# freemvmt/two-towers-overlords

Measured on NVIDIA B200. Metric: train_triplets_per_sec, higher is better.
Workload: dtype f32 (bf16x3 tensor-core projection)

## Files before the change

### two-towers-overlords_b200/csrc/tt_chain_sm100.cu

```cuda
#include <stdlib.h>

#include "tt_ptx.cuh"
#include "tt_step_ws.cuh"
#include "tt_tma.cuh"

namespace tt {

namespace {

using namespace ptx;

constexpr int BM = 128, BN = 128, BK = 64;
constexpr int kMaxStages = 6;
constexpr int kAcc = 4;
constexpr int kEpiThreads = 256;
constexpr int kThreads = 64 + kEpiThreads;
constexpr uint32_t kABytes = BM * BK * 2, kBBytes = BN * BK * 2, kStageBytes = kABytes + kBBytes;
constexpr int kSplitPad = 66;
constexpr int kRowStage = 3072;
constexpr int kTermPitch = 48;
constexpr int kTermBlock = 32 * kTermPitch;
constexpr int kF32Pitch = 80;
constexpr int kCsBytes = 2 * 8 * 64 * 4;
constexpr int kStagingBytes = kCsBytes  + 8 * kRowStage  + 64;
static_assert(2 * 64 * kSplitPad * 2 <= 8 * kRowStage, "split tiles overlay the row staging");
constexpr size_t chain_smem(int stages) { return (size_t)stages * kStageBytes + 1024 + 256 + kStagingBytes; }
constexpr float kCosEps = 1e-8f;
constexpr long long kSpinLimit = 4000000000ll;

enum { T_S = 0, T_T, T_F1, T_F2L, T_DZ, T_DX, T_DW2, T_DW1, T_G, T_COUNT };

struct TowerMaps {
  CUtensorMap x[3], w1[3];
  CUtensorMap h[2], w2[2];
  CUtensorMap dy[2];
  CUtensorMap dz[2], w1k[2];
  CUtensorMap dyk[2], hk[2];
  CUtensorMap dzk[2], xk[2];
};

struct SplitJobC {
  const float* X;
  bf16 *hi, *lo, *lo2;
  int R, C;
  int f4_0;
};

struct alignas(64) ChainParams {
  TowerMaps tm[2];
  int B, H, P, RTB, NC, NCH, NCF;
  int pairs, terms, pairs1, terms1;
  int kcb, nch[2], kbt[2];
  int off[T_COUNT + 1];
  int stages, n_sj, n_split_f4, n_split_f4_w1;
  int nS;
  int use_pdl;
  SplitJobC sj[6];
  float margin, inv_batch, grad_scale;
  const float *b1[2], *b2[2];
  float *h, *y, *dy, *dz1, *dxhat, *stats, *loss;
  bf16 *h_hi, *h_lo, *dy_hi, *dy_lo, *dz_hi, *dz_lo;
  float *part2, *part1;
  float *dW1[2], *db1[2], *dW2[2], *db2[2];
  float *stat_part, *cs1, *cs2, *hinge_part, *ybuf;
  unsigned* ctr;
  int n_counters;
  double* adam_state;
  float *adam_p, *adam_g, *adam_m, *adam_v;
  float lr, beta1, beta2, eps;
  int grad_accumulate;
  unsigned total_signals, dw2_signals;
  unsigned long long* trace;
};

__device__ __forceinline__ unsigned ld_acquire(const unsigned* p) {
  unsigned v;
  asm volatile("ld.acquire.gpu.global.u32 %0, [%1];" : "=r"(v) : "l"(p) : "memory");
  return v;
}
// ... 34 lines not shown
};
__device__ __forceinline__ RowTile row_tile(const ChainParams& p, int u) {
  RowTile rt;
  rt.r = u / 3;
  rt.seg = u - 3 * rt.r;
  rt.t = rt.seg != 0;
  rt.trow = (rt.seg == 2 ? p.B : 0) + rt.r * BM;
  rt.grow = rt.seg * p.B + rt.r * BM;
  rt.valid = min(BM, p.B - rt.r * BM);
  return rt;
}

struct Sub {
  const CUtensorMap *a, *b;
  int terms, pairs, m0, n0, kb0, nkb;
  int bn;
  int amn, bmn;
};
__device__ __forceinline__ int n_subs(int type) {
  return (type == T_S || type == T_T || type == T_G) ? 0 : 1;
}

__device__ __forceinline__ void dw_chunk(const ChainParams& p, int ci, int& t, int& j) {
  t = ci >= p.nch[0];
  j = ci - (t ? p.nch[0] : 0);
}

__device__ __forceinline__ Sub get_sub(const ChainParams& p, Task tk, int k) {
  Sub s;
  s.terms = p.terms;
  s.pairs = p.pairs;
  s.kb0 = 0;
  s.bn = BN;
  s.amn = s.bmn = 0;
  switch (tk.type) {
    case T_F1: {
      const RowTile rt = row_tile(p, tk.i / p.NC);
      s.a = p.tm[rt.t].x; s.b = p.tm[rt.t].w1;
      s.terms = p.terms1; s.pairs = p.pairs1;
      s.m0 = rt.trow; s.n0 = (tk.i % p.NC) * BN; s.nkb = p.H / BK;
    } break;
    case T_F2L: {
      const int seg = tk.i % 3, rc = tk.i / 3, r = rc / p.NCF, t = seg != 0;
      s.a = p.tm[t].h; s.b = p.tm[t].w2;
      s.m0 = (seg == 2 ? p.B : 0) + r * BM; s.n0 = (rc % p.NCF) * 64; s.nkb = p.P / BK;
      s.bn = 64;
    } break;
    case T_DZ: {
      const RowTile rt = row_tile(p, tk.i / p.NC);
      s.a = p.tm[rt.t].dy; s.b = p.tm[rt.t].w2; s.bmn = 1;
      s.m0 = rt.trow; s.n0 = (tk.i % p.NC) * BN; s.nkb = p.P / BK;
    } break;
    case T_DX: {
      const RowTile rt = row_tile(p, tk.i / p.NCH);
      s.a = p.tm[rt.t].dz; s.b = p.tm[rt.t].w1k; s.bmn = 1;
      s.m0 = rt.trow; s.n0 = (tk.i % p.NCH) * BN; s.nkb = p.P / BK;
    } break;
    case T_DW2: {
      const int nt_ = p.NC * p.NC, tile = tk.i % nt_;
      int t, j;
      dw_chunk(p, tk.i / nt_, t, j);
      s.a = p.tm[t].dyk; s.b = p.tm[t].hk; s.amn = s.bmn = 1;
      s.m0 = (tile / p.NC) * BM; s.n0 = (tile % p.NC) * BN;
      s.kb0 = j * p.kcb; s.nkb = min(p.kcb, p.kbt[t] - s.kb0);
    } break;
    default: {
      const int nt_ = p.NC * p.NCH, tile = tk.i % nt_;
      int t, j;
      dw_chunk(p, tk.i / nt_, t, j);
      s.a = p.tm[t].dzk; s.b = p.tm[t].xk; s.amn = s.bmn = 1;
      s.m0 = (tile / p.NCH) * BM; s.n0 = (tile % p.NCH) * BN;
      s.kb0 = j * p.kcb; s.nkb = min(p.kcb, p.kbt[t] - s.kb0);
    } break;
  }
  return s;
}

__device__ __forceinline__ unsigned* h_ready(const ChainParams& p) { return p.ctr + 8; }
__device__ __forceinline__ unsigned* dy_ready(const ChainParams& p) { return p.ctr + 8 + 3 * p.RTB; }
__device__ __forceinline__ unsigned* dz_ready(const ChainParams& p) { return p.ctr + 8 + 6 * p.RTB; }
__device__ __forceinline__ unsigned* stat_ready(const ChainParams& p) { return p.ctr + 8 + 9 * p.RTB; }
__device__ __forceinline__ unsigned* y_ready(const ChainParams& p) { return p.ctr + 8 + 10 * p.RTB; }

__device__ __forceinline__ void wait_rows(const ChainParams& p, const unsigned* ready, unsigned need, int t, int k0,
                                          int k1) {
  if (t == 0) {
    for (int r = k0 / BM; r <= (k1 - 1) / BM; ++r) wait_counter(ready + r, need);
    return;
  }
  if (k0 < p.B)
    for (int r = k0 / BM; r <= (min(k1, p.B) - 1) / BM; ++r) wait_counter(ready + p.RTB + r, need);
  if (k1 > p.B)
    for (int r = (max(k0, p.B) - p.B) / BM; r <= (k1 - p.B - 1) / BM; ++r) wait_counter(ready + 2 * p.RTB + r, need);
}

__device__ __forceinline__ void wait_deps(const ChainParams& p, Task tk) {
  switch (tk.type) {
    case T_F1: wait_counter(p.ctr + 0, (unsigned)p.nS); break;
    case T_F2L: {
      const int seg = tk.i % 3, r = tk.i / 3 / p.NCF;
      wait_counter(p.ctr + 2, (unsigned)p.nS);
      wait_counter(h_ready(p) + seg * p.RTB + r, p.NC);
    } break;
    case T_DZ: {
      const RowTile rt = row_tile(p, tk.i / p.NC);
      wait_counter(dy_ready(p) + rt.seg * p.RTB + rt.r, p.NCF);
    } break;
    case T_DX: {
      const RowTile rt = row_tile(p, tk.i / p.NCH);
      wait_counter(dz_ready(p) + rt.seg * p.RTB + rt.r, p.NC);
    } break;
    case T_DW2:
    case T_DW1: {
      const int nt_ = tk.type == T_DW2 ? p.NC * p.NC : p.NC * p.NCH;
      int t, j;
      dw_chunk(p, tk.i / nt_, t, j);
      const int k0 = j * p.kcb * BK, k1 = min(k0 + p.kcb * BK, t ? 2 * p.B : p.B);
      if (tk.type == T_DW2) wait_rows(p, dy_ready(p), p.NCF, t, k0, k1);
      else wait_rows(p, dz_ready(p), p.NC, t, k0, k1);
    } break;
    default: break;
  }
}

__device__ __forceinline__ float colsum16(const float (&v)[16], int lane) {
  float a[8], b[4], c[2];
  const bool h16 = lane & 16, h8 = lane & 8, h4 = lane & 4, h2 = lane & 2;
#pragma unroll
  for (int j = 0; j < 8; ++j) {
    const float keep = h16 ? v[8 + j] : v[j], send = h16 ? v[j] : v[8 + j];
    a[j] = keep + __shfl_xor_sync(0xffffffffu, send, 16);
  }
#pragma unroll
// ... 82 lines not shown
  e.ab += n;
  if (e.ab >= kAcc) {
    e.ab -= kAcc;
    e.aph ^= 1u;
  }
}
__device__ __forceinline__ void publish(const EpiCtx& e) {
  fence_proxy_async();
  __threadfence();
  epi_bar();
}

__device__ __forceinline__ void stage_cs(const EpiCtx& e, int slot, int chunk, float d) {
  if ((e.lane & 1) == 0) e.cs_s[(slot * 8 + e.we) * 64 + chunk * 16 + (e.lane >> 1)] = d;
}
__device__ __forceinline__ float reduce_cs(const EpiCtx& e, int slot, int col, int cw = 64) {
  const int hf = col / cw, cc = col - hf * cw;
  float s = 0.f;
#pragma unroll
  for (int quarter = 0; quarter < 4; ++quarter) s += e.cs_s[(slot * 8 + hf * 4 + ((quarter - 2) & 3)) * 64 + cc];
  return s;
}

__device__ __forceinline__ uint32_t pack_bf16(bf16 a, bf16 b) {
  return (uint32_t)__bfloat16_as_ushort(a) | ((uint32_t)__bfloat16_as_ushort(b) << 16);
}

__device__ void epi_split(const ChainParams& p, EpiCtx& e, int task_i) {
  const int nS = p.nS;
  if (task_i == 0 && e.tid == 0 && p.adam_state) {
    const double t = p.adam_state[0];
    p.adam_state[0] = t + 1.0;
// ... 73 lines not shown
    stage16(e.rs, e.lane, hi);
    stage16(e.rs + kTermBlock, e.lane, lo);
    if (ok && p.h) store16(p.h + (wrow0 + e.lane) * p.P + n, v);
    __syncwarp();
    flush16(e.rs, e.lane, p.h_hi, wrow0, n, p.P, vr);
    flush16(e.rs + kTermBlock, e.lane, p.h_lo, wrow0, n, p.P, vr);
    __syncwarp();
  }
  tc_fence_before();
  mbar_arrive(&e.acc_empty[e.ab]);
  acc_advance(e, 1);
  publish(e);
  if (e.tid == 0) signal(h_ready(p) + rt.seg * p.RTB + rt.r);
}

__device__ void epi_f2l(const ChainParams& p, EpiCtx& e, int task_i) {
  const int seg = task_i % 3, rc = task_i / 3, r = rc / p.NCF, c = rc % p.NCF, n0 = c * 64;
  const int valid = min(BM, p.B - r * BM);
  const int row = e.q * 32 + e.lane;
  const bool ok = row < valid;
  const int vr = warp_valid_rows(e, valid);
  const int trip = r * BM + row;
  const size_t wrow0 = (size_t)seg * p.B + (size_t)r * BM + e.q * 32;
  mbar_wait(&e.acc_full[e.ab], e.aph);
  tc_fence_after();
  trace_ev(e, 2);
  const uint32_t accb = e.tmem_base + ((uint32_t)(e.q * 32) << 16) + (uint32_t)(e.ab * BN + e.hf * 32);
  const float* bias = p.b2[seg != 0];
  float* X = p.ybuf + (size_t)rc * 3 * 64 * 128;
  float own[32];
#pragma unroll
  for (int ch = 0; ch < 2; ++ch) {
    const int col = e.hf * 32 + ch * 16;
    float v[16];
    tmem_ld16(accb + ch * 16, v);
#pragma unroll
    for (int j = 0; j < 16; ++j) {
      v[j] += __ldg(bias + n0 + col + j);
      own[ch * 16 + j] = v[j];
      X[((size_t)(seg * 64 + col + j)) * 128 + row] = v[j];
    }
    if (p.y && ok) store16(p.y + ((size_t)seg * p.B + trip) * p.P + n0 + col, v);
  }
  tc_fence_before();
  mbar_arrive(&e.acc_empty[e.ab]);
  acc_advance(e, 1);
  __threadfence();
  epi_bar();
  if (e.tid == 0) {
    signal(y_ready(p) + rc);
    wait_counter(y_ready(p) + rc, 3u);
  }
  epi_bar();
  const int s1 = seg == 0 ? 1 : 0, s2 = seg == 2 ? 1 : 2;
  float f1[32], f2[32];
  {
    const float* x1 = X + (size_t)(s1 * 64 + e.hf * 32) * 128 + row;
    const float* x2 = X + (size_t)(s2 * 64 + e.hf * 32) * 128 + row;
#pragma unroll
    for (int j = 0; j < 32; ++j) {
      f1[j] = __ldcg(x1 + (size_t)j * 128);
      f2[j] = __ldcg(x2 + (size_t)j * 128);
    }
  }
  float qq = 0.f, pp = 0.f, nn = 0.f, qp = 0.f, qn = 0.f;
#pragma unroll
  for (int j = 0; j < 32; ++j) {
    const float a = seg == 0 ? own[j] : f1[j];
    const float b = seg == 0 ? f1[j] : (seg == 1 ? own[j] : f2[j]);
    const float d = seg == 2 ? own[j] : f2[j];
    qq = fmaf(a, a, qq);
    pp = fmaf(b, b, pp);
    nn = fmaf(d, d, nn);
    qp = fmaf(a, b, qp);
    qn = fmaf(a, d, qn);
  }
  const int nslots = p.NCF;
  float* xs = e.cs_s;
  if (seg == 0 && e.hf == 1) {
    xs[row] = qq; xs[128 + row] = pp; xs[256 + row] = nn; xs[384 + row] = qp; xs[512 + row] = qn;
  }
  epi_bar();
  if (seg == 0 && e.hf == 0) {
    float* sp = p.stat_part + ((size_t)(r * nslots + c) * 5) * 128 + row;
    sp[0] = qq + xs[row]; sp[128] = pp + xs[128 + row]; sp[256] = nn + xs[256 + row]; sp[384] = qp + xs[384 + row];
    sp[512] = qn + xs[512 + row];
    __threadfence();
  }
  epi_bar();
  if (e.tid == 0) {
    if (seg == 0) signal(stat_ready(p) + r);
    wait_counter(stat_ready(p) + r, (unsigned)p.NCF);
  }
  epi_bar();
  trace_ev(e, 3);
  qq = pp = nn = qp = qn = 0.f;
  for (int s0 = 0; s0 < nslots; s0 += 4) {
    float v[4][5];
#pragma unroll
    for (int u = 0; u < 4; ++u) {
      const float* sp = p.stat_part + ((size_t)(r * nslots + min(s0 + u, nslots - 1)) * 5) * 128 + row;
#pragma unroll
      for (int w = 0; w < 5; ++w) v[u][w] = __ldcg(sp + 128 * w);
    }
#pragma unroll
    for (int u = 0; u < 4; ++u)
      if (s0 + u < nslots) {
        qq += v[u][0]; pp += v[u][1]; nn += v[u][2]; qp += v[u][3]; qn += v[u][4];
      }
  }
  const float nq = sqrtf(qq), np_ = sqrtf(pp), nn_ = sqrtf(nn);
  const float cq = fmaxf(nq, kCosEps), cp = fmaxf(np_, kCosEps), cn = fmaxf(nn_, kCosEps);
  const float cos_p = qp / (cq * cp), cos_n = qn / (cq * cn);
  const float hinge = ok ? fmaxf((1.f - cos_p) - (1.f - cos_n) + p.margin, 0.f) : 0.f;
  const float gh = (hinge > 0.f) ? p.grad_scale * p.inv_batch : 0.f;
  const float a_qp = -gh / (cq * cp), a_qn = gh / (cq * cn);
  float c_own, c1, c2;
  if (seg == 0) {
    c_own = -((nq > kCosEps) ? (-gh * cos_p + gh * cos_n) / (cq * nq) : 0.f); c1 = a_qp; c2 = a_qn;
  } else if (seg == 1) {
    c_own = -((np_ > kCosEps) ? (-gh * cos_p) / (cp * np_) : 0.f); c1 = a_qp; c2 = 0.f;
  } else {
    c_own = -((nn_ > kCosEps) ? (gh * cos_n) / (cn * nn_) : 0.f); c1 = a_qn; c2 = 0.f;
  }
  if (seg == 0 && c == 0 && e.hf == 0) {
    if (ok) {
      float* s = p.stats + (size_t)trip * 8;
      s[0] = cos_p; s[1] = cos_n; s[2] = hinge; s[3] = nq; s[4] = np_; s[5] = nn_; s[6] = qp; s[7] = qn;
    }
    const float hsum = warp_sum(hinge);
    if (e.lane == 0) e.hs_s[e.q] = hsum;
  }
  uint8_t* blk_hi = e.rs;
  uint8_t* blk_lo = e.rs + kTermBlock;
#pragma unroll
  for (int ch = 0; ch < 2; ++ch) {
    const int n = n0 + e.hf * 32 + ch * 16;
    float g[16];
#pragma unroll
    for (int j = 0; j < 16; ++j)
      g[j] = ok ? (c_own * own[ch * 16 + j] + c1 * f1[ch * 16 + j] + c2 * f2[ch * 16 + j]) : 0.f;
    alignas(16) bf16 hi[16], lo[16];
    split16(g, hi, lo);
    stage16(blk_hi, e.lane, hi);
    stage16(blk_lo, e.lane, lo);
    if (ok && p.dy) store16(p.dy + ((size_t)seg * p.B + trip) * p.P + n, g);
    __syncwarp();
    flush16(blk_hi, e.lane, p.dy_hi, wrow0, n, p.P, vr);
    flush16(blk_lo, e.lane, p.dy_lo, wrow0, n, p.P, vr);
    __syncwarp();
    stage_cs(e, 0, ch, colsum16(g, e.lane));
  }
  epi_bar();
  if (e.tid < 64) p.cs2[(size_t)(seg * p.RTB + r) * p.P + n0 + e.tid] = reduce_cs(e, 0, e.tid, 32);
  if (seg == 0 && c == 0 && e.tid == 0) p.hinge_part[r] = (e.hs_s[0] + e.hs_s[1]) + (e.hs_s[2] + e.hs_s[3]);
  publish(e);
  if (e.tid == 0) {
    signal(dy_ready(p) + seg * p.RTB + r);
    signal(p.ctr + 1);
  }
}

__device__ void epi_dz(const ChainParams& p, EpiCtx& e, int task_i) {
  const RowTile rt = row_tile(p, task_i / p.NC);
  const int n0 = (task_i % p.NC) * BN;
  mbar_wait(&e.acc_full[e.ab], e.aph);
  tc_fence_after();
  trace_ev(e, 2);
  const int row = e.q * 32 + e.lane;
  const bool ok = row < rt.valid;
  const int vr = warp_valid_rows(e, rt.valid);
  const size_t wrow0 = (size_t)rt.grow + e.q * 32;
  for (int ch = 0; ch < 4; ++ch) {
// ... 173 lines not shown
            if (j + c4 < nch[u]) acc[u] = add4(acc[u], t[u][c4]);
      }
      emit4(p, k, dst[0], acc[0]);
      if (two) emit4(p, k, dst[1], acc[1]);
    }
  };
  sum_pairs(p.ctr + 6, p.part2, p.dW2, (size_t)p.P * p.P / 4);
  if (e.tid == 0) wait_counter(p.ctr + 1, p.total_signals);
  epi_bar();
  sum_pairs(p.ctr + 7, p.part1, p.dW1, (size_t)p.P * p.H / 4);
  {
    const int nout = 4 * p.P;
    const int gw = task_i * 8 + e.we, nw = nG * 8;
    for (int o = gw; o < nout; o += nw) {
      const int which = o / p.P, n = o - which * p.P, t = which & 1;
      const float* src;
      int cnt;
      if (which < 2) {
        src = p.cs2 + (size_t)(t ? p.RTB : 0) * p.P + n;
        cnt = t ? 2 * p.RTB : p.RTB;
      } else {
        src = p.cs1 + (size_t)(t ? p.RTB : 0) * p.P + n;
        cnt = t ? 2 * p.RTB : p.RTB;
      }
      float s = 0.f;
      for (int r = e.lane; r < cnt; r += 32) s += __ldcg(src + (size_t)r * p.P);
      s = warp_sum(s);
      if (e.lane == 0) emit1(p, k, (which < 2 ? p.db2[t] : p.db1[t]) + n, s);
    }
  }
  if (task_i == 0 && e.tid == 0) {
    float s = 0.f;
    for (int r = 0; r < p.RTB; ++r) s += __ldcg(p.hinge_part + r);
    *p.loss = s * p.inv_batch;
  }
  epi_bar();
  if (e.tid == 0) {
    __threadfence();
    if (atomicAdd(p.ctr + 4, 1u) == (unsigned)nG - 1u) {
      for (int i = 0; i < p.n_counters; ++i) p.ctr[i] = 0u;
    }
  }
}

__global__ void __launch_bounds__(kThreads, 1) chain_kernel(const __grid_constant__ ChainParams p) {
  extern __shared__ uint8_t smem_raw[];
  const int warp = threadIdx.x >> 5, lane = threadIdx.x & 31;
  const uint32_t raw = smem_u32(smem_raw);
// ... 31 lines not shown
    if (elect_one()) {
      int s = 0;
      uint32_t ph = 0;
      if (p.use_pdl) pdl_wait();
      for (int idx = blockIdx.x; idx < n_tasks; idx += gridDim.x) {
        const Task tk = decode(p, idx);
        const int ns = n_subs(tk.type);
        if (ns == 0) continue;
        wait_deps(p, tk);
        fence_proxy_async();
        for (int k = 0; k < ns; ++k) {
          const Sub sb = get_sub(p, tk, k);
          for (int kb = sb.kb0; kb < sb.kb0 + sb.nkb; ++kb) {
            for (int j = 0; j < sb.terms; ++j) {
              mbar_wait(&empty[s], ph ^ 1u);
              mbar_arrive_expect_tx(&full[s], kABytes + (uint32_t)sb.bn * BK * 2);
              uint8_t* sa = smem + s * kStageBytes;
              uint8_t* sbm = sa + kABytes;
              if (sb.amn) {
                tma_load_2d(sa, &sb.a[j], &full[s], sb.m0, kb * BK);
                tma_load_2d(sa + kABytes / 2, &sb.a[j], &full[s], sb.m0 + 64, kb * BK);
              } else {
                tma_load_2d(sa, &sb.a[j], &full[s], kb * BK, sb.m0);
              }
              if (sb.bmn) {
                tma_load_2d(sbm, &sb.b[j], &full[s], sb.n0, kb * BK);
                tma_load_2d(sbm + kBBytes / 2, &sb.b[j], &full[s], sb.n0 + 64, kb * BK);
              } else {
                tma_load_2d(sbm, &sb.b[j], &full[s], kb * BK, sb.n0);
              }
              if (++s == NS) {
                s = 0;
                ph ^= 1u;
              }
            }
          }
        }
      }
    }
  } else if (warp == 1) {
    if (elect_one()) {
      constexpr uint32_t idesc128 = make_idesc_bf16(BM, BN), idesc64 = make_idesc_bf16(BM, 64);
      const uint32_t ring = smem_u32(smem);
      int s = 0, ab = 0;
      uint32_t ph = 0, aph = 0;
      for (int idx = blockIdx.x; idx < n_tasks; idx += gridDim.x) {
        const Task tk = decode(p, idx);
        const int ns = n_subs(tk.type);
        for (int k = 0; k < ns; ++k) {
          const Sub sb = get_sub(p, tk, k);
          const uint32_t idesc = (sb.bn == BN ? idesc128 : idesc64) | ((uint32_t)sb.amn << 15) | ((uint32_t)sb.bmn << 16);
          const uint64_t a_step = sb.amn ? 128 : 2, b_step = sb.bmn ? 128 : 2;
          mbar_wait(&acc_empty[ab], aph ^ 1u);
          tc_fence_after();
          const uint32_t acc = tmem_base + (uint32_t)(ab * BN);
          for (int kbi = 0; kbi < sb.nkb; ++kbi) {
            uint32_t slot_addr[3];
            int slot_id[3];
            for (int j = 0; j < sb.terms; ++j) {
              mbar_wait(&full[s], ph);
              slot_id[j] = s;
              slot_addr[j] = ring + (uint32_t)s * kStageBytes;
              if (++s == NS) {
                s = 0;
                ph ^= 1u;
              }
// ... 34 lines not shown
    e.tid = threadIdx.x - 64;
    e.ab = 0;
    e.aph = 0;
    e.trace = p.trace ? p.trace + (size_t)blockIdx.x * kTraceSlots * 2 : nullptr;
    e.tslot = 0;
    for (int idx = blockIdx.x; idx < n_tasks; idx += gridDim.x) {
      const Task tk = decode(p, idx);
      e.tidx = idx;
      trace_ev(e, 0);
      switch (tk.type) {
        case T_S:
          epi_split(p, e, tk.i);
          if (p.use_pdl) pdl_wait();
          break;
        case T_F1: epi_f1(p, e, tk.i); break;
        case T_F2L: epi_f2l(p, e, tk.i); break;
        case T_DZ: epi_dz(p, e, tk.i); break;
        case T_DX: epi_dx(p, e, tk.i); break;
        case T_DW2:
        case T_DW1: epi_dw(p, e, tk); break;
        default: epi_grad(p, e, tk.i); break;
      }
      trace_ev(e, 1);
    }
  }
  tc_fence_before();
  __syncthreads();
  if (warp == 1) tmem_dealloc(tmem_base, kAcc * BN);
}

constexpr int kChainStages = 5;
// ... 37 lines not shown
  const float* W2[2] = {s.Wq2, s.Wd2};
  const int row0[2] = {0, B}, rows[2] = {B, 2 * B};
  const bool x3 = s.n_split == 3;
  for (int t = 0; t < 2; ++t) {
    TowerMaps& m = p.tm[t];
    const size_t oH = (size_t)row0[t] * H, oP = (size_t)row0[t] * P;
    const bf16* x[3] = {w.x_hi + oH, x3 ? w.x_lo + oH : nullptr, x3 ? w.x_lo2 + oH : nullptr};
    const bf16* w1[3] = {w.w1_hi[t], w.w1_lo[t], w.w1_lo2[t]};
    const bf16* hh[2] = {w.h_hi + oP, w.h_lo + oP};
    const bf16* w2[2] = {w.w2_hi[t], w.w2_lo[t]};
    const bf16* dy[2] = {w.dy_hi + oP, w.dy_lo + oP};
    const bf16* dz[2] = {w.dz_hi + oP, w.dz_lo + oP};
    if ((rc = map_terms(m.x, 3, x, rows[t], H, H))) return rc;
    if ((rc = map_terms(m.w1, 3, w1, P, H, H))) return rc;
    if ((rc = map_terms(m.h, 2, hh, rows[t], P, P))) return rc;
    if ((rc = map_terms(m.w2, 2, w2, P, P, P, 64))) return rc;
    if ((rc = map_terms(m.dy, 2, dy, rows[t], P, P))) return rc;
    if ((rc = map_terms(m.dz, 2, dz, rows[t], P, P))) return rc;
    if ((rc = map_terms(m.w1k, 2, w1, P, H, H, 64))) return rc;
    if ((rc = map_terms(m.dyk, 2, dy, rows[t], P, P, 64))) return rc;
    if ((rc = map_terms(m.hk, 2, hh, rows[t], P, P, 64))) return rc;
    if ((rc = map_terms(m.dzk, 2, dz, rows[t], P, P, 64))) return rc;
    if ((rc = map_terms(m.xk, 2, x, rows[t], H, H, 64))) return rc;
  }
  p.B = B; p.H = H; p.P = P;
  p.RTB = (B + BM - 1) / BM; p.NC = (P + BN - 1) / BN; p.NCH = (H + BN - 1) / BN; p.NCF = P / 64;
  p.pairs = x3 ? 3 : 1; p.terms = x3 ? 2 : 1;
  p.pairs1 = x3 ? 6 : 1; p.terms1 = x3 ? 3 : 1;
  for (int t = 0; t < 2; ++t) p.kbt[t] = (rows[t] + BK - 1) / BK;
  p.kcb = 8;
  {
    const char* e = getenv("TT_CHAIN_KCB");
    if (e && atoi(e) >= 4) p.kcb = atoi(e) / 4 * 4;
  }
  while ((p.kbt[0] + p.kcb - 1) / p.kcb + (p.kbt[1] + p.kcb - 1) / p.kcb > 48) p.kcb += 8;
  for (int t = 0; t < 2; ++t) p.nch[t] = (p.kbt[t] + p.kcb - 1) / p.kcb;
  const int grid = sm_count();
  TT_REQUIRE(grid >= 3 * (P / 64), "tt_triplet_step: projection dim %d needs %d co-resident CTAs, the device has %d SMs", P,
             3 * (P / 64), grid);
  const int n_rt = 3 * p.RTB, nchs = p.nch[0] + p.nch[1];
  const int count[T_COUNT] = {grid,
                              0,
                              n_rt * p.NC,
                              n_rt * p.NCF,
                              n_rt * p.NC,
                              s.dxhat ? n_rt * p.NCH : 0,
                              nchs * p.NC * p.NC,
                              nchs * p.NC * p.NCH,
                              grid};
  p.off[0] = 0;
  for (int k = 0; k < T_COUNT; ++k) p.off[k + 1] = p.off[k] + count[k];
  p.total_signals = (unsigned)(count[T_F2L] + count[T_DZ] + count[T_DW2] + count[T_DW1]);
  p.dw2_signals = (unsigned)count[T_DW2];
  p.stages = kChainStages;
  int f4 = 0;
  p.n_sj = 0;
  for (int t = 0; t < 2; ++t) {
    p.sj[p.n_sj++] = SplitJobC{W1[t], w.w1_hi[t], w.w1_lo[t], x3 ? w.w1_lo2[t] : nullptr, P, H, f4};
    f4 += P * H / 4;
  }
  p.n_split_f4_w1 = f4;
  for (int t = 0; t < 2; ++t) {
    p.sj[p.n_sj++] = SplitJobC{W2[t], w.w2_hi[t], w.w2_lo[t], nullptr, P, P, f4};
    f4 += P * P / 4;
  }
  p.n_split_f4 = f4;
  p.margin = s.margin; p.inv_batch = s.inv_batch; p.grad_scale = s.grad_scale;
  p.b1[0] = s.bq1; p.b1[1] = s.bd1; p.b2[0] = s.bq2; p.b2[1] = s.bd2;
  const bool dbg = chain_debug_out() != 0;
  p.h = dbg ? s.h : nullptr; p.y = dbg ? s.y : nullptr; p.dy = dbg ? s.dy : nullptr; p.dz1 = dbg ? w.dz1 : nullptr;
  p.dxhat = s.dxhat; p.stats = s.stats; p.loss = s.loss;
  p.h_hi = w.h_hi; p.h_lo = w.h_lo;
  p.dy_hi = w.dy_hi; p.dy_lo = w.dy_lo;
  p.dz_hi = w.dz_hi; p.dz_lo = w.dz_lo;
  p.part2 = w.partial2; p.part1 = w.partial;
  p.dW1[0] = s.dWq1; p.dW1[1] = s.dWd1; p.db1[0] = s.dbq1; p.db1[1] = s.dbd1;
  p.dW2[0] = s.dWq2; p.dW2[1] = s.dWd2; p.db2[0] = s.dbq2; p.db2[1] = s.dbd2;
  p.stat_part = w.stat_part; p.cs1 = w.cs1; p.cs2 = w.cs2; p.hinge_part = w.hinge_part; p.ybuf = w.ybuf;
  p.ctr = w.counters;
  p.n_counters = w.n_counters;
  p.nS = grid;
  p.grad_accumulate = s.grad_accumulate;
  if (s.adam.param) {
    const FusedAdam& a = s.adam;
    TT_REQUIRE(a.state && a.grad && a.exp_avg && a.exp_avg_sq, "tt_triplet_step: fused Adam needs state, grad and both moments");
    const float* W[8] = {s.Wq1, s.bq1, s.Wq2, s.bq2, s.Wd1, s.bd1, s.Wd2, s.bd2};
    float* G[8] = {s.dWq1, s.dbq1, s.dWq2, s.dbq2, s.dWd1, s.dbd1, s.dWd2, s.dbd2};
    const size_t len[8] = {(size_t)P * H, (size_t)P, (size_t)P * P, (size_t)P, (size_t)P * H, (size_t)P, (size_t)P * P, (size_t)P};
    for (int i = 0; i < 8; ++i) {
      const ptrdiff_t off = G[i] - a.grad;
      TT_REQUIRE(off >= 0 && (size_t)off + len[i] <= a.n && W[i] == a.param + off && off % 4 == 0,
                 "tt_triplet_step: fused Adam wants the 8 projection tensors and their gradients to be slices of the "
                 "flat buffers at equal, 16-byte aligned offsets (tensor %d)", i);
// ... 27 lines not shown
```

### two-towers-overlords_b200/csrc/tt_step_ws.cuh

```cuda
#pragma once
#include "tt_simt.cuh"
#include "tt_sm100.cuh"

namespace tt {

using bf16 = __nv_bfloat16;
static inline int round64(int x) { return (x + 63) / 64 * 64; }

struct StepWs {
  int ldt, dcol;
  bf16 *x_hi, *x_lo, *x_lo2, *xt_hi, *xt_lo;
  bf16 *h_hi, *h_lo, *ht_hi, *ht_lo;
  bf16 *dy_hi, *dy_lo, *dyt_hi, *dyt_lo;
  bf16 *dz_hi, *dz_lo, *dzt_hi, *dzt_lo;
  bf16 *w1_hi[2], *w1_lo[2], *w1_lo2[2], *w1t_hi[2], *w1t_lo[2];
  bf16 *w2_hi[2], *w2_lo[2], *w2t_hi[2], *w2t_lo[2];
  float *dz1, *partial, *partial2, *colsum, *colsum2, *loss_scratch;
  float *stat_part, *cs1, *cs2, *hinge_part, *ybuf;
  unsigned* counters;
  int n_counters;
  unsigned long long* trace;
};
constexpr int kTraceSlots = 64, kTraceCtas = 160;

static inline size_t carve_step(char* base, int B, int H, int P, int train_table, StepWs* out) {
  char* p = base;
  StepWs w{};
  w.dcol = round64(B);
  w.ldt = w.dcol + round64(2 * B);
  const size_t R = (size_t)3 * B;
  w.x_hi = ws_take<bf16>(p, R * H); w.x_lo = ws_take<bf16>(p, R * H); w.x_lo2 = ws_take<bf16>(p, R * H);
  w.xt_hi = ws_take<bf16>(p, (size_t)H * w.ldt); w.xt_lo = ws_take<bf16>(p, (size_t)H * w.ldt);
  w.h_hi = ws_take<bf16>(p, R * P); w.h_lo = ws_take<bf16>(p, R * P);
// ... 4 lines not shown
  w.dzt_hi = ws_take<bf16>(p, (size_t)P * w.ldt); w.dzt_lo = ws_take<bf16>(p, (size_t)P * w.ldt);
  for (int t = 0; t < 2; ++t) {
    w.w1_hi[t] = ws_take<bf16>(p, (size_t)P * H); w.w1_lo[t] = ws_take<bf16>(p, (size_t)P * H);
    w.w1_lo2[t] = ws_take<bf16>(p, (size_t)P * H);
    w.w1t_hi[t] = ws_take<bf16>(p, (size_t)P * H); w.w1t_lo[t] = ws_take<bf16>(p, (size_t)P * H);
    w.w2_hi[t] = ws_take<bf16>(p, (size_t)P * P); w.w2_lo[t] = ws_take<bf16>(p, (size_t)P * P);
    w.w2t_hi[t] = ws_take<bf16>(p, (size_t)P * P); w.w2t_lo[t] = ws_take<bf16>(p, (size_t)P * P);
  }
  w.dz1 = ws_take<float>(p, R * P);
  w.partial = ws_take<float>(p, (size_t)2 * 32 * P * max(P, H));
  w.partial2 = ws_take<float>(p, (size_t)2 * 32 * P * P);
  w.colsum = ws_take<float>(p, (size_t)2 * kColsumSlices * P);
  w.colsum2 = ws_take<float>(p, (size_t)2 * kColsumSlices * P);
  w.loss_scratch = ws_take<float>(p, (size_t)(B + 3) / 4 + 8);
  {
    const int RTB = (B + 127) / 128, NC = (P + 127) / 128;
    w.stat_part = ws_take<float>(p, (size_t)RTB * 2 * (P / 64 + 1) * 5 * 128);
    w.cs1 = ws_take<float>(p, (size_t)3 * RTB * P);
    w.cs2 = ws_take<float>(p, (size_t)3 * RTB * P);
    w.ybuf = ws_take<float>(p, (size_t)3 * RTB * 128 * P);
    w.hinge_part = ws_take<float>(p, (size_t)RTB + 8);
    w.n_counters = 10 * RTB + 8 + RTB * (P / 64 + 1);
    w.counters = ws_take<unsigned>(p, (size_t)w.n_counters);
    w.trace = ws_take<unsigned long long>(p, (size_t)kTraceCtas * kTraceSlots * 2);
  }
  (void)train_table;
  if (out) *out = w;
  return (size_t)(p - base) + 256;
}


}
```

Baseline: 8.511 million.

## Split fused F2+loss task into separate F2 GEMM and per-row-block loss tasks

Replaces the fused F2L task (64-wide N tiles that exchanged y across CTAs and spun on per-row-block statistic barriers) with a plain 128-wide F2 GEMM that writes y to a column-major buffer, plus a separate loss task. The loss task waits on all three segments, reduces norms and dot products in shared memory, and emits dy for all three segments, with each row block split into quarter-row and column-part pieces. This removes the cross-CTA spin waits inside the epilogue and the need for 3*(P/64) co-resident CTAs, and it moves F2 to full 128-wide MMA tiles. In exchange the loss tasks reread y from global memory and column sums gain a fourth partial dimension.

Result: no change. 8.538 million, median of 6 (+0.3%).

```diff
diff --git a/two-towers-overlords_b200/csrc/tt_chain_sm100.cu b/two-towers-overlords_b200/csrc/tt_chain_sm100.cu
--- a/two-towers-overlords_b200/csrc/tt_chain_sm100.cu
+++ b/two-towers-overlords_b200/csrc/tt_chain_sm100.cu
@@ -27,13 +27,15 @@
 constexpr size_t chain_smem(int stages) { return (size_t)stages * kStageBytes + 1024 + 256 + kStagingBytes; }
 constexpr float kCosEps = 1e-8f;
 constexpr long long kSpinLimit = 4000000000ll;
-
-enum { T_S = 0, T_T, T_F1, T_F2L, T_DZ, T_DX, T_DW2, T_DW1, T_G, T_COUNT };
+constexpr int kLCP = 2, kLPR = 4 * kLCP;
+static_assert(5 * 8 * 32 * 4 <= 8 * kRowStage, "a round of loss statistics overlays the row staging");
+
+enum { T_S = 0, T_T, T_F1, T_F2, T_L, T_DZ, T_DX, T_DW2, T_DW1, T_G, T_COUNT };
 
 struct TowerMaps {
   CUtensorMap x[3], w1[3];
   CUtensorMap h[2], w2[2];
-  CUtensorMap dy[2];
+  CUtensorMap dy[2], w2k[2];
   CUtensorMap dz[2], w1k[2];
   CUtensorMap dyk[2], hk[2];
   CUtensorMap dzk[2], xk[2];
@@ -48,7 +50,7 @@
 
 struct alignas(64) ChainParams {
   TowerMaps tm[2];
-  int B, H, P, RTB, NC, NCH, NCF;
+  int B, H, P, RTB, NC, NCH;
   int pairs, terms, pairs1, terms1;
   int kcb, nch[2], kbt[2];
   int off[T_COUNT + 1];
@@ -62,7 +64,8 @@
   bf16 *h_hi, *h_lo, *dy_hi, *dy_lo, *dz_hi, *dz_lo;
   float *part2, *part1;
   float *dW1[2], *db1[2], *dW2[2], *db2[2];
-  float *stat_part, *cs1, *cs2, *hinge_part, *ybuf;
+  float *cs1, *cs2, *hinge_part;
+  float* ybuf;
   unsigned* ctr;
   int n_counters;
   double* adam_state;
@@ -127,11 +130,10 @@
 struct Sub {
   const CUtensorMap *a, *b;
   int terms, pairs, m0, n0, kb0, nkb;
-  int bn;
   int amn, bmn;
 };
 __device__ __forceinline__ int n_subs(int type) {
-  return (type == T_S || type == T_T || type == T_G) ? 0 : 1;
+  return (type == T_S || type == T_T || type == T_L || type == T_G) ? 0 : 1;
 }
 
 __device__ __forceinline__ void dw_chunk(const ChainParams& p, int ci, int& t, int& j) {
@@ -144,7 +146,6 @@
   s.terms = p.terms;
   s.pairs = p.pairs;
   s.kb0 = 0;
-  s.bn = BN;
   s.amn = s.bmn = 0;
   switch (tk.type) {
     case T_F1: {
@@ -153,15 +154,14 @@
       s.terms = p.terms1; s.pairs = p.pairs1;
       s.m0 = rt.trow; s.n0 = (tk.i % p.NC) * BN; s.nkb = p.H / BK;
     } break;
-    case T_F2L: {
-      const int seg = tk.i % 3, rc = tk.i / 3, r = rc / p.NCF, t = seg != 0;
-      s.a = p.tm[t].h; s.b = p.tm[t].w2;
-      s.m0 = (seg == 2 ? p.B : 0) + r * BM; s.n0 = (rc % p.NCF) * 64; s.nkb = p.P / BK;
-      s.bn = 64;
+    case T_F2: {
+      const RowTile rt = row_tile(p, tk.i / p.NC);
+      s.a = p.tm[rt.t].h; s.b = p.tm[rt.t].w2;
+      s.m0 = rt.trow; s.n0 = (tk.i % p.NC) * BN; s.nkb = p.P / BK;
     } break;
     case T_DZ: {
       const RowTile rt = row_tile(p, tk.i / p.NC);
-      s.a = p.tm[rt.t].dy; s.b = p.tm[rt.t].w2; s.bmn = 1;
+      s.a = p.tm[rt.t].dy; s.b = p.tm[rt.t].w2k; s.bmn = 1;
       s.m0 = rt.trow; s.n0 = (tk.i % p.NC) * BN; s.nkb = p.P / BK;
     } break;
     case T_DX: {
@@ -192,8 +192,7 @@
 __device__ __forceinline__ unsigned* h_ready(const ChainParams& p) { return p.ctr + 8; }
 __device__ __forceinline__ unsigned* dy_ready(const ChainParams& p) { return p.ctr + 8 + 3 * p.RTB; }
 __device__ __forceinline__ unsigned* dz_ready(const ChainParams& p) { return p.ctr + 8 + 6 * p.RTB; }
-__device__ __forceinline__ unsigned* stat_ready(const ChainParams& p) { return p.ctr + 8 + 9 * p.RTB; }
-__device__ __forceinline__ unsigned* y_ready(const ChainParams& p) { return p.ctr + 8 + 10 * p.RTB; }
+__device__ __forceinline__ unsigned* y_ready(const ChainParams& p) { return p.ctr + 8 + 9 * p.RTB; }
 
 __device__ __forceinline__ void wait_rows(const ChainParams& p, const unsigned* ready, unsigned need, int t, int k0,
                                           int k1) {
@@ -210,14 +209,14 @@
 __device__ __forceinline__ void wait_deps(const ChainParams& p, Task tk) {
   switch (tk.type) {
     case T_F1: wait_counter(p.ctr + 0, (unsigned)p.nS); break;
-    case T_F2L: {
-      const int seg = tk.i % 3, r = tk.i / 3 / p.NCF;
+    case T_F2: {
+      const RowTile rt = row_tile(p, tk.i / p.NC);
       wait_counter(p.ctr + 2, (unsigned)p.nS);
-      wait_counter(h_ready(p) + seg * p.RTB + r, p.NC);
+      wait_counter(h_ready(p) + rt.seg * p.RTB + rt.r, p.NC);
     } break;
     case T_DZ: {
       const RowTile rt = row_tile(p, tk.i / p.NC);
-      wait_counter(dy_ready(p) + rt.seg * p.RTB + rt.r, p.NCF);
+      wait_counter(dy_ready(p) + rt.seg * p.RTB + rt.r, kLPR);
     } break;
     case T_DX: {
       const RowTile rt = row_tile(p, tk.i / p.NCH);
@@ -229,7 +228,7 @@
       int t, j;
       dw_chunk(p, tk.i / nt_, t, j);
       const int k0 = j * p.kcb * BK, k1 = min(k0 + p.kcb * BK, t ? 2 * p.B : p.B);
-      if (tk.type == T_DW2) wait_rows(p, dy_ready(p), p.NCF, t, k0, k1);
+      if (tk.type == T_DW2) wait_rows(p, dy_ready(p), kLPR, t, k0, k1);
       else wait_rows(p, dz_ready(p), p.NC, t, k0, k1);
     } break;
     default: break;
@@ -342,8 +341,8 @@
 __device__ __forceinline__ void stage_cs(const EpiCtx& e, int slot, int chunk, float d) {
   if ((e.lane & 1) == 0) e.cs_s[(slot * 8 + e.we) * 64 + chunk * 16 + (e.lane >> 1)] = d;
 }
-__device__ __forceinline__ float reduce_cs(const EpiCtx& e, int slot, int col, int cw = 64) {
-  const int hf = col / cw, cc = col - hf * cw;
+__device__ __forceinline__ float reduce_cs(const EpiCtx& e, int slot, int col) {
+  const int hf = col / 64, cc = col - hf * 64;
   float s = 0.f;
 #pragma unroll
   for (int quarter = 0; quarter < 4; ++quarter) s += e.cs_s[(slot * 8 + hf * 4 + ((quarter - 2) & 3)) * 64 + cc];
@@ -447,100 +446,91 @@
   if (e.tid == 0) signal(h_ready(p) + rt.seg * p.RTB + rt.r);
 }
 
-__device__ void epi_f2l(const ChainParams& p, EpiCtx& e, int task_i) {
-  const int seg = task_i % 3, rc = task_i / 3, r = rc / p.NCF, c = rc % p.NCF, n0 = c * 64;
-  const int valid = min(BM, p.B - r * BM);
-  const int row = e.q * 32 + e.lane;
-  const bool ok = row < valid;
-  const int vr = warp_valid_rows(e, valid);
-  const int trip = r * BM + row;
-  const size_t wrow0 = (size_t)seg * p.B + (size_t)r * BM + e.q * 32;
+__device__ void epi_f2(const ChainParams& p, EpiCtx& e, int task_i) {
+  const RowTile rt = row_tile(p, task_i / p.NC);
+  const int n0 = (task_i % p.NC) * BN;
   mbar_wait(&e.acc_full[e.ab], e.aph);
   tc_fence_after();
   trace_ev(e, 2);
-  const uint32_t accb = e.tmem_base + ((uint32_t)(e.q * 32) << 16) + (uint32_t)(e.ab * BN + e.hf * 32);
-  const float* bias = p.b2[seg != 0];
-  float* X = p.ybuf + (size_t)rc * 3 * 64 * 128;
-  float own[32];
-#pragma unroll
-  for (int ch = 0; ch < 2; ++ch) {
-    const int col = e.hf * 32 + ch * 16;
+  const int row = e.q * 32 + e.lane;
+  const bool ok = row < rt.valid;
+  const size_t ldy = (size_t)p.RTB * BM;
+  float* yb = p.ybuf + (size_t)rt.seg * p.P * ldy + (size_t)rt.r * BM + row;
+  const float* bias = p.b2[rt.t];
+  for (int ch = 0; ch < 4; ++ch) {
+    const int n = n0 + e.hf * 64 + ch * 16;
+    if (n >= p.P) break;
     float v[16];
-    tmem_ld16(accb + ch * 16, v);
+    tmem_ld16(acc_addr(e, e.ab, ch), v);
 #pragma unroll
     for (int j = 0; j < 16; ++j) {
-      v[j] += __ldg(bias + n0 + col + j);
-      own[ch * 16 + j] = v[j];
-      X[((size_t)(seg * 64 + col + j)) * 128 + row] = v[j];
-    }
-    if (p.y && ok) store16(p.y + ((size_t)seg * p.B + trip) * p.P + n0 + col, v);
+      v[j] += __ldg(bias + n + j);
+      yb[(size_t)(n + j) * ldy] = v[j];
+    }
+    if (ok && p.y) store16(p.y + ((size_t)rt.grow + row) * p.P + n, v);
   }
   tc_fence_before();
   mbar_arrive(&e.acc_empty[e.ab]);
   acc_advance(e, 1);
-  __threadfence();
+  publish(e);
+  if (e.tid == 0) signal(y_ready(p) + rt.seg * p.RTB + rt.r);
+}
+
+__device__ void epi_loss(const ChainParams& p, EpiCtx& e, int task_i) {
+  const int part = task_i % kLCP, qd = task_i / kLCP % 4, r = task_i / kLPR;
+  const int row = qd * 32 + e.lane, trip = r * BM + row;
+  const bool ok = trip < p.B;
+  const int vr = max(0, min(32, p.B - r * BM - qd * 32));
+  if (e.tid == 0)
+    for (int seg = 0; seg < 3; ++seg) wait_counter(y_ready(p) + seg * p.RTB + r, p.NC);
   epi_bar();
-  if (e.tid == 0) {
-    signal(y_ready(p) + rc);
-    wait_counter(y_ready(p) + rc, 3u);
-  }
-  epi_bar();
-  const int s1 = seg == 0 ? 1 : 0, s2 = seg == 2 ? 1 : 2;
-  float f1[32], f2[32];
-  {
-    const float* x1 = X + (size_t)(s1 * 64 + e.hf * 32) * 128 + row;
-    const float* x2 = X + (size_t)(s2 * 64 + e.hf * 32) * 128 + row;
-#pragma unroll
-    for (int j = 0; j < 32; ++j) {
-      f1[j] = __ldcg(x1 + (size_t)j * 128);
-      f2[j] = __ldcg(x2 + (size_t)j * 128);
-    }
-  }
+  trace_ev(e, 2);
+  const int nslot = p.P / 64;
+  const size_t ldy = (size_t)p.RTB * BM, segy = (size_t)p.P * ldy;
+  const float* yr = p.ybuf + (size_t)r * BM + row;
+  float* st_s = reinterpret_cast<float*>(e.sp_s);
   float qq = 0.f, pp = 0.f, nn = 0.f, qp = 0.f, qn = 0.f;
-#pragma unroll
-  for (int j = 0; j < 32; ++j) {
-    const float a = seg == 0 ? own[j] : f1[j];
-    const float b = seg == 0 ? f1[j] : (seg == 1 ? own[j] : f2[j]);
-    const float d = seg == 2 ? own[j] : f2[j];
-    qq = fmaf(a, a, qq);
-    pp = fmaf(b, b, pp);
-    nn = fmaf(d, d, nn);
-    qp = fmaf(a, b, qp);
-    qn = fmaf(a, d, qn);
-  }
-  const int nslots = p.NCF;
-  float* xs = e.cs_s;
-  if (seg == 0 && e.hf == 1) {
-    xs[row] = qq; xs[128 + row] = pp; xs[256 + row] = nn; xs[384 + row] = qp; xs[512 + row] = qn;
-  }
-  epi_bar();
-  if (seg == 0 && e.hf == 0) {
-    float* sp = p.stat_part + ((size_t)(r * nslots + c) * 5) * 128 + row;
-    sp[0] = qq + xs[row]; sp[128] = pp + xs[128 + row]; sp[256] = nn + xs[256 + row]; sp[384] = qp + xs[384 + row];
-    sp[512] = qn + xs[512 + row];
-    __threadfence();
-  }
-  epi_bar();
-  if (e.tid == 0) {
-    if (seg == 0) signal(stat_ready(p) + r);
-    wait_counter(stat_ready(p) + r, (unsigned)p.NCF);
-  }
-  epi_bar();
-  trace_ev(e, 3);
-  qq = pp = nn = qp = qn = 0.f;
-  for (int s0 = 0; s0 < nslots; s0 += 4) {
-    float v[4][5];
-#pragma unroll
-    for (int u = 0; u < 4; ++u) {
-      const float* sp = p.stat_part + ((size_t)(r * nslots + min(s0 + u, nslots - 1)) * 5) * 128 + row;
-#pragma unroll
-      for (int w = 0; w < 5; ++w) v[u][w] = __ldcg(sp + 128 * w);
-    }
-#pragma unroll
-    for (int u = 0; u < 4; ++u)
-      if (s0 + u < nslots) {
-        qq += v[u][0]; pp += v[u][1]; nn += v[u][2]; qp += v[u][3]; qn += v[u][4];
+  for (int s0 = 0; s0 < nslot; s0 += 8) {
+    const int s = s0 + e.we;
+    if (s < nslot) {
+      float v5[5];
+#pragma unroll
+      for (int hf = 0; hf < 2; ++hf) {
+        float sq = 0.f, sp = 0.f, sn = 0.f, sqp = 0.f, sqn = 0.f;
+#pragma unroll
+        for (int c16 = 0; c16 < 2; ++c16) {
+          const float* y0 = yr + (size_t)(s * 64 + hf * 32 + c16 * 16) * ldy;
+          float a[16], b[16], d[16];
+#pragma unroll
+          for (int j = 0; j < 16; ++j) {
+            a[j] = __ldcg(y0 + (size_t)j * ldy);
+            b[j] = __ldcg(y0 + segy + (size_t)j * ldy);
+            d[j] = __ldcg(y0 + 2 * segy + (size_t)j * ldy);
+          }
+#pragma unroll
+          for (int j = 0; j < 16; ++j) {
+            sq = fmaf(a[j], a[j], sq);
+            sp = fmaf(b[j], b[j], sp);
+            sn = fmaf(d[j], d[j], sn);
+            sqp = fmaf(a[j], b[j], sqp);
+            sqn = fmaf(a[j], d[j], sqn);
+          }
+        }
+        if (hf == 0) {
+          v5[0] = sq; v5[1] = sp; v5[2] = sn; v5[3] = sqp; v5[4] = sqn;
+        } else {
+          v5[0] = v5[0] + sq; v5[1] = v5[1] + sp; v5[2] = v5[2] + sn; v5[3] = v5[3] + sqp; v5[4] = v5[4] + sqn;
+        }
       }
+#pragma unroll
+      for (int w = 0; w < 5; ++w) st_s[(e.we * 5 + w) * 32 + e.lane] = v5[w];
+    }
+    epi_bar();
+    for (int u = 0; u < min(8, nslot - s0); ++u) {
+      const float* v = st_s + u * 5 * 32 + e.lane;
+      qq += v[0]; pp += v[32]; nn += v[64]; qp += v[96]; qn += v[128];
+    }
+    epi_bar();
   }
   const float nq = sqrtf(qq), np_ = sqrtf(pp), nn_ = sqrtf(nn);
   const float cq = fmaxf(nq, kCosEps), cp = fmaxf(np_, kCosEps), cn = fmaxf(nn_, kCosEps);
@@ -548,48 +538,52 @@
   const float hinge = ok ? fmaxf((1.f - cos_p) - (1.f - cos_n) + p.margin, 0.f) : 0.f;
   const float gh = (hinge > 0.f) ? p.grad_scale * p.inv_batch : 0.f;
   const float a_qp = -gh / (cq * cp), a_qn = gh / (cq * cn);
-  float c_own, c1, c2;
-  if (seg == 0) {
-    c_own = -((nq > kCosEps) ? (-gh * cos_p + gh * cos_n) / (cq * nq) : 0.f); c1 = a_qp; c2 = a_qn;
-  } else if (seg == 1) {
-    c_own = -((np_ > kCosEps) ? (-gh * cos_p) / (cp * np_) : 0.f); c1 = a_qp; c2 = 0.f;
-  } else {
-    c_own = -((nn_ > kCosEps) ? (gh * cos_n) / (cn * nn_) : 0.f); c1 = a_qn; c2 = 0.f;
-  }
-  if (seg == 0 && c == 0 && e.hf == 0) {
+  float c_own[3], c1[3], c2[3];
+  c_own[0] = -((nq > kCosEps) ? (-gh * cos_p + gh * cos_n) / (cq * nq) : 0.f); c1[0] = a_qp; c2[0] = a_qn;
+  c_own[1] = -((np_ > kCosEps) ? (-gh * cos_p) / (cp * np_) : 0.f); c1[1] = a_qp; c2[1] = 0.f;
+  c_own[2] = -((nn_ > kCosEps) ? (gh * cos_n) / (cn * nn_) : 0.f); c1[2] = a_qn; c2[2] = 0.f;
+  if (part == 0 && e.we == 0) {
     if (ok) {
-      float* s = p.stats + (size_t)trip * 8;
-      s[0] = cos_p; s[1] = cos_n; s[2] = hinge; s[3] = nq; s[4] = np_; s[5] = nn_; s[6] = qp; s[7] = qn;
+      float* st = p.stats + (size_t)trip * 8;
+      st[0] = cos_p; st[1] = cos_n; st[2] = hinge; st[3] = nq; st[4] = np_; st[5] = nn_; st[6] = qp; st[7] = qn;
     }
     const float hsum = warp_sum(hinge);
-    if (e.lane == 0) e.hs_s[e.q] = hsum;
+    if (e.lane == 0) p.hinge_part[r * 4 + qd] = hsum;
   }
   uint8_t* blk_hi = e.rs;
   uint8_t* blk_lo = e.rs + kTermBlock;
-#pragma unroll
-  for (int ch = 0; ch < 2; ++ch) {
-    const int n = n0 + e.hf * 32 + ch * 16;
-    float g[16];
-#pragma unroll
-    for (int j = 0; j < 16; ++j)
-      g[j] = ok ? (c_own * own[ch * 16 + j] + c1 * f1[ch * 16 + j] + c2 * f2[ch * 16 + j]) : 0.f;
-    alignas(16) bf16 hi[16], lo[16];
-    split16(g, hi, lo);
-    stage16(blk_hi, e.lane, hi);
-    stage16(blk_lo, e.lane, lo);
-    if (ok && p.dy) store16(p.dy + ((size_t)seg * p.B + trip) * p.P + n, g);
-    __syncwarp();
-    flush16(blk_hi, e.lane, p.dy_hi, wrow0, n, p.P, vr);
-    flush16(blk_lo, e.lane, p.dy_lo, wrow0, n, p.P, vr);
-    __syncwarp();
-    stage_cs(e, 0, ch, colsum16(g, e.lane));
-  }
-  epi_bar();
-  if (e.tid < 64) p.cs2[(size_t)(seg * p.RTB + r) * p.P + n0 + e.tid] = reduce_cs(e, 0, e.tid, 32);
-  if (seg == 0 && c == 0 && e.tid == 0) p.hinge_part[r] = (e.hs_s[0] + e.hs_s[1]) + (e.hs_s[2] + e.hs_s[3]);
+  const int nc16 = p.P / 16;
+  for (int c16 = part * nc16 / kLCP + e.we; c16 < (part + 1) * nc16 / kLCP; c16 += 8) {
+    const int n = c16 * 16;
+    float y3[3][16];
+#pragma unroll
+    for (int sg = 0; sg < 3; ++sg)
+#pragma unroll
+      for (int j = 0; j < 16; ++j) y3[sg][j] = __ldcg(yr + sg * segy + (size_t)(n + j) * ldy);
+#pragma unroll
+    for (int seg = 0; seg < 3; ++seg) {
+      const int s1 = seg == 0 ? 1 : 0, s2 = seg == 2 ? 1 : 2;
+      float g[16];
+#pragma unroll
+      for (int j = 0; j < 16; ++j)
+        g[j] = ok ? __fmaf_rn(c2[seg], y3[s2][j], __fmaf_rn(c_own[seg], y3[seg][j], __fmul_rn(c1[seg], y3[s1][j]))) : 0.f;
+      alignas(16) bf16 hi[16], lo[16];
+      split16(g, hi, lo);
+      stage16(blk_hi, e.lane, hi);
+      stage16(blk_lo, e.lane, lo);
+      if (ok && p.dy) store16(p.dy + ((size_t)seg * p.B + trip) * p.P + n, g);
+      __syncwarp();
+      const size_t wrow0 = (size_t)seg * p.B + (size_t)r * BM + qd * 32;
+      flush16(blk_hi, e.lane, p.dy_hi, wrow0, n, p.P, vr);
+      flush16(blk_lo, e.lane, p.dy_lo, wrow0, n, p.P, vr);
+      __syncwarp();
+      const float cs = colsum16(g, e.lane);
+      if ((e.lane & 1) == 0) p.cs2[((size_t)(seg * p.RTB + r) * 4 + qd) * p.P + n + (e.lane >> 1)] = cs;
+    }
+  }
   publish(e);
   if (e.tid == 0) {
-    signal(dy_ready(p) + seg * p.RTB + r);
+    for (int seg = 0; seg < 3; ++seg) signal(dy_ready(p) + seg * p.RTB + r);
     signal(p.ctr + 1);
   }
 }
@@ -793,24 +787,30 @@
     const int gw = task_i * 8 + e.we, nw = nG * 8;
     for (int o = gw; o < nout; o += nw) {
       const int which = o / p.P, n = o - which * p.P, t = which & 1;
-      const float* src;
-      int cnt;
+      const int cnt = t ? 2 * p.RTB : p.RTB;
+      float s = 0.f;
       if (which < 2) {
-        src = p.cs2 + (size_t)(t ? p.RTB : 0) * p.P + n;
-        cnt = t ? 2 * p.RTB : p.RTB;
+        const float* src = p.cs2 + (size_t)(t ? p.RTB : 0) * 4 * p.P + n;
+        for (int r = e.lane; r < cnt; r += 32) {
+          float v = 0.f;
+#pragma unroll
+          for (int qd = 0; qd < 4; ++qd) v += __ldcg(src + (size_t)(4 * r + qd) * p.P);
+          s += v;
+        }
       } else {
-        src = p.cs1 + (size_t)(t ? p.RTB : 0) * p.P + n;
-        cnt = t ? 2 * p.RTB : p.RTB;
+        const float* src = p.cs1 + (size_t)(t ? p.RTB : 0) * p.P + n;
+        for (int r = e.lane; r < cnt; r += 32) s += __ldcg(src + (size_t)r * p.P);
       }
-      float s = 0.f;
-      for (int r = e.lane; r < cnt; r += 32) s += __ldcg(src + (size_t)r * p.P);
       s = warp_sum(s);
       if (e.lane == 0) emit1(p, k, (which < 2 ? p.db2[t] : p.db1[t]) + n, s);
     }
   }
   if (task_i == 0 && e.tid == 0) {
     float s = 0.f;
-    for (int r = 0; r < p.RTB; ++r) s += __ldcg(p.hinge_part + r);
+    for (int r = 0; r < p.RTB; ++r) {
+      const float* h = p.hinge_part + 4 * r;
+      s += (__ldcg(h) + __ldcg(h + 1)) + (__ldcg(h + 2) + __ldcg(h + 3));
+    }
     *p.loss = s * p.inv_batch;
   }
   epi_bar();
@@ -872,7 +872,7 @@
           for (int kb = sb.kb0; kb < sb.kb0 + sb.nkb; ++kb) {
             for (int j = 0; j < sb.terms; ++j) {
               mbar_wait(&empty[s], ph ^ 1u);
-              mbar_arrive_expect_tx(&full[s], kABytes + (uint32_t)sb.bn * BK * 2);
+              mbar_arrive_expect_tx(&full[s], kStageBytes);
               uint8_t* sa = smem + s * kStageBytes;
               uint8_t* sbm = sa + kABytes;
               if (sb.amn) {
@@ -898,7 +898,7 @@
     }
   } else if (warp == 1) {
     if (elect_one()) {
-      constexpr uint32_t idesc128 = make_idesc_bf16(BM, BN), idesc64 = make_idesc_bf16(BM, 64);
+      constexpr uint32_t idesc128 = make_idesc_bf16(BM, BN);
       const uint32_t ring = smem_u32(smem);
       int s = 0, ab = 0;
       uint32_t ph = 0, aph = 0;
@@ -907,7 +907,7 @@
         const int ns = n_subs(tk.type);
         for (int k = 0; k < ns; ++k) {
           const Sub sb = get_sub(p, tk, k);
-          const uint32_t idesc = (sb.bn == BN ? idesc128 : idesc64) | ((uint32_t)sb.amn << 15) | ((uint32_t)sb.bmn << 16);
+          const uint32_t idesc = idesc128 | ((uint32_t)sb.amn << 15) | ((uint32_t)sb.bmn << 16);
           const uint64_t a_step = sb.amn ? 128 : 2, b_step = sb.bmn ? 128 : 2;
           mbar_wait(&acc_empty[ab], aph ^ 1u);
           tc_fence_after();
@@ -972,7 +972,8 @@
           if (p.use_pdl) pdl_wait();
           break;
         case T_F1: epi_f1(p, e, tk.i); break;
-        case T_F2L: epi_f2l(p, e, tk.i); break;
+        case T_F2: epi_f2(p, e, tk.i); break;
+        case T_L: epi_loss(p, e, tk.i); break;
         case T_DZ: epi_dz(p, e, tk.i); break;
         case T_DX: epi_dx(p, e, tk.i); break;
         case T_DW2:
@@ -1040,17 +1041,18 @@
     if ((rc = map_terms(m.x, 3, x, rows[t], H, H))) return rc;
     if ((rc = map_terms(m.w1, 3, w1, P, H, H))) return rc;
     if ((rc = map_terms(m.h, 2, hh, rows[t], P, P))) return rc;
-    if ((rc = map_terms(m.w2, 2, w2, P, P, P, 64))) return rc;
+    if ((rc = map_terms(m.w2, 2, w2, P, P, P))) return rc;
     if ((rc = map_terms(m.dy, 2, dy, rows[t], P, P))) return rc;
     if ((rc = map_terms(m.dz, 2, dz, rows[t], P, P))) return rc;
     if ((rc = map_terms(m.w1k, 2, w1, P, H, H, 64))) return rc;
+    if ((rc = map_terms(m.w2k, 2, w2, P, P, P, 64))) return rc;
     if ((rc = map_terms(m.dyk, 2, dy, rows[t], P, P, 64))) return rc;
     if ((rc = map_terms(m.hk, 2, hh, rows[t], P, P, 64))) return rc;
     if ((rc = map_terms(m.dzk, 2, dz, rows[t], P, P, 64))) return rc;
     if ((rc = map_terms(m.xk, 2, x, rows[t], H, H, 64))) return rc;
   }
   p.B = B; p.H = H; p.P = P;
-  p.RTB = (B + BM - 1) / BM; p.NC = (P + BN - 1) / BN; p.NCH = (H + BN - 1) / BN; p.NCF = P / 64;
+  p.RTB = (B + BM - 1) / BM; p.NC = (P + BN - 1) / BN; p.NCH = (H + BN - 1) / BN;
   p.pairs = x3 ? 3 : 1; p.terms = x3 ? 2 : 1;
   p.pairs1 = x3 ? 6 : 1; p.terms1 = x3 ? 3 : 1;
   for (int t = 0; t < 2; ++t) p.kbt[t] = (rows[t] + BK - 1) / BK;
@@ -1062,13 +1064,12 @@
   while ((p.kbt[0] + p.kcb - 1) / p.kcb + (p.kbt[1] + p.kcb - 1) / p.kcb > 48) p.kcb += 8;
   for (int t = 0; t < 2; ++t) p.nch[t] = (p.kbt[t] + p.kcb - 1) / p.kcb;
   const int grid = sm_count();
-  TT_REQUIRE(grid >= 3 * (P / 64), "tt_triplet_step: projection dim %d needs %d co-resident CTAs, the device has %d SMs", P,
-             3 * (P / 64), grid);
   const int n_rt = 3 * p.RTB, nchs = p.nch[0] + p.nch[1];
   const int count[T_COUNT] = {grid,
                               0,
                               n_rt * p.NC,
-                              n_rt * p.NCF,
+                              n_rt * p.NC,
+                              p.RTB * kLPR,
                               n_rt * p.NC,
                               s.dxhat ? n_rt * p.NCH : 0,
                               nchs * p.NC * p.NC,
@@ -1076,7 +1077,7 @@
                               grid};
   p.off[0] = 0;
   for (int k = 0; k < T_COUNT; ++k) p.off[k + 1] = p.off[k] + count[k];
-  p.total_signals = (unsigned)(count[T_F2L] + count[T_DZ] + count[T_DW2] + count[T_DW1]);
+  p.total_signals = (unsigned)(count[T_L] + count[T_DZ] + count[T_DW2] + count[T_DW1]);
   p.dw2_signals = (unsigned)count[T_DW2];
   p.stages = kChainStages;
   int f4 = 0;
@@ -1102,7 +1103,7 @@
   p.part2 = w.partial2; p.part1 = w.partial;
   p.dW1[0] = s.dWq1; p.dW1[1] = s.dWd1; p.db1[0] = s.dbq1; p.db1[1] = s.dbd1;
   p.dW2[0] = s.dWq2; p.dW2[1] = s.dWd2; p.db2[0] = s.dbq2; p.db2[1] = s.dbd2;
-  p.stat_part = w.stat_part; p.cs1 = w.cs1; p.cs2 = w.cs2; p.hinge_part = w.hinge_part; p.ybuf = w.ybuf;
+  p.cs1 = w.cs1; p.cs2 = w.cs2; p.hinge_part = w.hinge_part; p.ybuf = w.ybuf;
   p.ctr = w.counters;
   p.n_counters = w.n_counters;
   p.nS = grid;
diff --git a/two-towers-overlords_b200/csrc/tt_step_ws.cuh b/two-towers-overlords_b200/csrc/tt_step_ws.cuh
--- a/two-towers-overlords_b200/csrc/tt_step_ws.cuh
+++ b/two-towers-overlords_b200/csrc/tt_step_ws.cuh
@@ -16,7 +16,7 @@
   bf16 *w1_hi[2], *w1_lo[2], *w1_lo2[2], *w1t_hi[2], *w1t_lo[2];
   bf16 *w2_hi[2], *w2_lo[2], *w2t_hi[2], *w2t_lo[2];
   float *dz1, *partial, *partial2, *colsum, *colsum2, *loss_scratch;
-  float *stat_part, *cs1, *cs2, *hinge_part, *ybuf;
+  float *cs1, *cs2, *hinge_part, *ybuf;
   unsigned* counters;
   int n_counters;
   unsigned long long* trace;
@@ -51,13 +51,12 @@
   w.colsum2 = ws_take<float>(p, (size_t)2 * kColsumSlices * P);
   w.loss_scratch = ws_take<float>(p, (size_t)(B + 3) / 4 + 8);
   {
-    const int RTB = (B + 127) / 128, NC = (P + 127) / 128;
-    w.stat_part = ws_take<float>(p, (size_t)RTB * 2 * (P / 64 + 1) * 5 * 128);
+    const int RTB = (B + 127) / 128;
     w.cs1 = ws_take<float>(p, (size_t)3 * RTB * P);
-    w.cs2 = ws_take<float>(p, (size_t)3 * RTB * P);
+    w.cs2 = ws_take<float>(p, (size_t)3 * RTB * 4 * P);
     w.ybuf = ws_take<float>(p, (size_t)3 * RTB * 128 * P);
-    w.hinge_part = ws_take<float>(p, (size_t)RTB + 8);
-    w.n_counters = 10 * RTB + 8 + RTB * (P / 64 + 1);
+    w.hinge_part = ws_take<float>(p, (size_t)4 * RTB + 8);
+    w.n_counters = 12 * RTB + 8;
     w.counters = ws_take<unsigned>(p, (size_t)w.n_counters);
     w.trace = ws_take<unsigned long long>(p, (size_t)kTraceCtas * kTraceSlots * 2);
   }
```
